# NVlabs/UnseenObjectClustering

Measured on AMD Instinct MI355X. Metric: frames/sec at 640x480 RGB-D, two-stage clustering, higher is better.
Workload: dtype f32; 1 GPU; configs[3] frames: full two-stage (crop-and-refine) segmentation of single 640x480 RGB-D frames; throughput schedule 3 streams x 4-frame launch sets (one frame at a time: `latency`); frame=640x480, seeds=100, iters=10, crop=224, total_frames=513, frames_per_gpu=513, collective=False, frames_in_flight_per_gpu=12, streams_per_gpu=3, frames_per_launch=4

## Files before the change

include/uoc_hip.h:

```cpp
#ifndef UOC_HIP_H
#define UOC_HIP_H

#include <stddef.h>
#include <stdint.h>

#ifdef __cplusplus
extern "C" {
#endif

#define UOC_OK 0
#define UOC_EINVAL (-22)
#define UOC_ENOMEM (-12)
#define UOC_EHIP (-5)
#define UOC_ENOENT (-2)
#define UOC_ETIMEDOUT (-110)

#define UOC_EMBED_DIM 64
#define UOC_MAX_SEEDS 128
#define UOC_METRIC_COSINE 0
#define UOC_METRIC_EUCLIDEAN 1

int uoc_version(void);
int uoc_is_dev_build(void);
unsigned long long uoc_config_fingerprint(void);
// ... 45 lines not shown
                     size_t ws_bytes, void *stream);
int uoc_ms_cluster_ex(const float *d_X, int batch, int n, int m, float kappa, int iters, float epsilon, int metric,
                      const int32_t *d_first_index, int32_t *d_labels, int32_t *d_indices, float *d_Z_out,
                      int32_t *d_seed_labels_out, void *d_ws, size_t ws_bytes, void *stream);
int uoc_ms_cluster_wide_ex(const float *d_X, int halves, int batch, int n, int m, float kappa, int iters, float epsilon,
                           int metric, const int32_t *d_first_index, int32_t *d_labels, int32_t *d_indices, float *d_Z_out,
                           int32_t *d_seed_labels_out, void *d_ws, size_t ws_bytes, void *stream);


typedef struct uoc_net uoc_net;

enum { UOC_NET_RGBD_ADD = 0, UOC_NET_COLOR = 1, UOC_NET_DEPTH = 2, UOC_NET_RGBD_EARLY = 3, UOC_NET_RGBD_CAT = 4 };

int uoc_net_create(uoc_net **out);
int uoc_net_create_mode(uoc_net **out, int mode);
int uoc_net_embed_dim(const uoc_net *net);
int uoc_net_destroy(uoc_net *net);
int uoc_net_load_param(uoc_net *net, const char *name, const float *host_data, size_t numel);
int uoc_net_finalize(uoc_net *net);
size_t uoc_net_workspace_bytes(const uoc_net *net, int B, int H, int W);
int uoc_net_set_split_precision(uoc_net *net, int on);
int uoc_net_forward(uoc_net *net, const float *d_rgb, const float *d_xyz, int B, int H, int W, float *d_embed,
                    void *d_ws, size_t ws_bytes, void *stream);

#define UOC_CONV_DIRECT 0
#define UOC_CONV_WINOGRAD4 4
#define UOC_CONV_WINOGRAD4_BF16X3 5
int uoc_conv2d_nhwc(const float *d_in, const float *d_w, const float *d_bias, const float *d_res, float *d_out,
                    int G, int B, int H, int W, int Cin, int Cout, int K, int stride, int dil, int pad, int relu,
                    void *stream);
int uoc_conv2d_nhwc_algo(const float *d_in, const float *d_w, const float *d_bias, const float *d_res, float *d_out,
                         int G, int B, int H, int W, int Cin, int Cout, int K, int stride, int dil, int pad, int relu,
                         int algo, void *stream);


typedef struct uoc_roi_table {
  int32_t K;
  int32_t label[128];
  int32_t box[128][4];
} uoc_roi_table;

size_t uoc_roi_workspace_bytes(void);

int uoc_prep_rgbd(const uint8_t *d_bgr, const uint16_t *d_depth_mm, int H, int W, float fx, float fy, float px,
                  float py, float mean_b, float mean_g, float mean_r, float *d_image, float *d_xyz, void *stream);

int uoc_filter_labels_depth(int32_t *d_labels, const float *d_z, long z_batch_stride, int B, int H, int W,
                            float threshold, void *d_ws, size_t ws_bytes, void *stream);

int uoc_roi_build(int32_t *d_labels, const float *d_z, int H, int W, float threshold, float pad_fraction,
                  uoc_roi_table *d_table, void *d_ws, size_t ws_bytes, void *stream);

int uoc_roi_crop(const float *d_rgb, const float *d_xyz, const int32_t *d_labels, int H, int W,
                 const uoc_roi_table *d_table, int K, int S, float *d_rgb_crops, float *d_xyz_crops,
                 float *d_mask_crops, void *stream);

int uoc_roi_match_stats(const int32_t *d_labels_crop, const float *d_mask_crops, const float *d_xyz_crops, int K,
                        int S, int32_t *d_keep, float *d_meanz, void *d_ws, size_t ws_bytes, void *stream);

int uoc_roi_paste(const int32_t *d_labels_crop, const uoc_roi_table *d_table, const int32_t *d_map,
                  const int32_t *d_order, int K, int S, int H, int W, int32_t *d_refined, void *stream);

int uoc_roi_match(const int32_t *d_labels_crop, const float *d_mask_crops, const float *d_xyz_crops,
                  const uoc_roi_table *d_table, int K, int S, int H, int W, int32_t *d_refined, int32_t *d_keep,
                  int32_t *d_plan, int32_t *d_status, void *d_ws, size_t ws_bytes, void *stream);

// ... 172 lines not shown
```

unseenobjectclustering_amd/_native.py:

```python
from __future__ import annotations

import ctypes
import os
from ctypes import c_char_p, c_float, c_int, c_int32, c_size_t, c_void_p, POINTER

from .build import LIB_PATH

_lib = None


class NativeError(RuntimeError):
    pass


def _declare(lib):
    P = c_void_p
    lib.uoc_version.restype = c_int
    lib.uoc_is_dev_build.argtypes = []
    lib.uoc_is_dev_build.restype = c_int
    lib.uoc_config_fingerprint.argtypes = []
    lib.uoc_config_fingerprint.restype = ctypes.c_ulonglong
    lib.uoc_shutdown.restype = c_int
    lib.uoc_reload_env.argtypes = []
    lib.uoc_reload_env.restype = c_int
# ... 13 lines not shown
    lib.uoc_ms_seed_components.argtypes = [P, c_int, c_int, c_float, P, P, P]
    lib.uoc_ms_assign.argtypes = [P, c_int, c_int, P, P, P, c_int, P, P, P, c_size_t, P]
    lib.uoc_ms_cluster.argtypes = [P, c_int, c_int, c_int, c_float, c_int, c_float, P, P, P, P, P, P, c_size_t, P]
    lib.uoc_ms_check.argtypes = [P]
    lib.uoc_ms_check.restype = c_int
    lib.uoc_ms_workspace_bytes_wide.restype = c_size_t
    lib.uoc_ms_workspace_bytes_wide.argtypes = [c_int, c_int, c_int, c_int]
    lib.uoc_ms_cluster_wide.argtypes = [P, c_int, c_int, c_int, c_int, c_float, c_int, c_float, P, P, P, P, P, P, c_size_t, P]
    lib.uoc_ms_cluster_wide.restype = c_int
    lib.uoc_ms_select_seeds_ex.argtypes = [P, c_int, c_int, c_int, c_int, P, P, P, c_int, P, c_size_t, P]
    lib.uoc_ms_hill_climb_ex.argtypes = [P, c_int, c_int, P, c_int, c_float, c_int, c_int, P, c_size_t, P]
    lib.uoc_ms_seed_components_ex.argtypes = [P, c_int, c_int, c_float, c_int, P, P, P]
    lib.uoc_ms_assign_ex.argtypes = [P, c_int, c_int, P, P, P, c_int, c_int, P, P, P, c_size_t, P]
    lib.uoc_ms_cluster_ex.argtypes = [P, c_int, c_int, c_int, c_float, c_int, c_float, c_int, P, P, P, P, P, P, c_size_t, P]
    lib.uoc_ms_cluster_wide_ex.argtypes = [P, c_int, c_int, c_int, c_int, c_float, c_int, c_float, c_int, P, P, P, P, P, P,
                                           c_size_t, P]
    for name in METRIC_SYMBOLS:
        getattr(lib, name).restype = c_int
    lib.uoc_net_embed_dim.argtypes = [P]
    lib.uoc_net_embed_dim.restype = c_int
    lib.uoc_net_create.argtypes = [POINTER(P)]
    lib.uoc_net_create_mode.argtypes = [POINTER(P), c_int]
    lib.uoc_net_destroy.argtypes = [P]
    lib.uoc_net_load_param.argtypes = [P, c_char_p, P, c_size_t]
    lib.uoc_net_finalize.argtypes = [P]
    lib.uoc_net_workspace_bytes.restype = c_size_t
    lib.uoc_net_workspace_bytes.argtypes = [P, c_int, c_int, c_int]
    lib.uoc_net_forward.argtypes = [P, P, P, c_int, c_int, c_int, P, P, c_size_t, P]
    lib.uoc_net_set_split_precision.argtypes = [P, c_int]
    lib.uoc_net_set_split_precision.restype = c_int
    lib.uoc_conv2d_nhwc.argtypes = [P, P, P, P, P] + [c_int] * 11 + [P]
    lib.uoc_conv2d_nhwc_algo.argtypes = [P, P, P, P, P] + [c_int] * 12 + [P]
    lib.uoc_conv2d_nhwc_algo.restype = c_int
    for name in ("uoc_net_create", "uoc_net_create_mode", "uoc_net_destroy", "uoc_net_load_param", "uoc_net_finalize", "uoc_net_forward",
                 "uoc_conv2d_nhwc"):
        getattr(lib, name).restype = c_int
    lib.uoc_eval_workspace_bytes.restype = c_size_t
    lib.uoc_eval_workspace_bytes.argtypes = [c_int, c_int]
    lib.uoc_eval_pair_stats.argtypes = [P, P, c_int, c_int, c_int, P, P, c_size_t, P]
    lib.uoc_eval_pair_stats.restype = c_int
    lib.uoc_roi_workspace_bytes.restype = c_size_t
    lib.uoc_roi_workspace_bytes.argtypes = []
    lib.uoc_prep_rgbd.argtypes = [P, P, c_int, c_int] + [c_float] * 7 + [P, P, P]
    lib.uoc_prep_rgbd.restype = c_int
    lib.uoc_filter_labels_depth.argtypes = [P, P, ctypes.c_long, c_int, c_int, c_int, c_float, P, c_size_t, P]
    lib.uoc_roi_build.argtypes = [P, P, c_int, c_int, c_float, c_float, P, P, c_size_t, P]
    lib.uoc_roi_crop.argtypes = [P, P, P, c_int, c_int, P, c_int, c_int, P, P, P, P]
    lib.uoc_roi_match_stats.argtypes = [P, P, P, c_int, c_int, P, P, P, c_size_t, P]
    lib.uoc_roi_paste.argtypes = [P, P, P, P, c_int, c_int, c_int, c_int, P, P]
    lib.uoc_labels_to_u8.argtypes = [P, ctypes.c_long, P, P, P]
    lib.uoc_roi_match.argtypes = [P, P, P, P, c_int, c_int, c_int, c_int, P, P, P, P, P, c_size_t, P]
    for name in ("uoc_filter_labels_depth", "uoc_roi_build", "uoc_roi_crop", "uoc_roi_match_stats", "uoc_roi_paste", "uoc_labels_to_u8", "uoc_roi_match"):
        getattr(lib, name).restype = c_int
    lib.uoc_objects_workspace_bytes.argtypes = [c_int, c_int, c_int]
    lib.uoc_objects_workspace_bytes.restype = c_size_t
    lib.uoc_objects.argtypes = [P, P, P, c_int, c_int, c_int, c_int, c_int, P, P, P, P, ctypes.c_long, P, P, c_size_t, P]
    lib.uoc_objects.restype = c_int
    lib.uoc_track_state_bytes.argtypes = [c_int, c_int, c_int]
    lib.uoc_track_state_bytes.restype = c_size_t
    lib.uoc_track_workspace_bytes.argtypes = [c_int]
    lib.uoc_track_workspace_bytes.restype = c_size_t
    lib.uoc_track_reset.argtypes = [P, c_int, c_int, c_int, c_int, P]
    lib.uoc_track_reset.restype = c_int
    lib.uoc_track_step.argtypes = [P, c_int, c_int, c_int, c_int, c_int, P, P, P, P, P, c_size_t, P]
    lib.uoc_track_step.restype = c_int
    lib.uoc_cc_workspace_bytes.argtypes = [c_int, c_int, c_int]
# ... 26 lines not shown
    lib.uoc_footprint.restype = c_int
    lib.uoc_lzf_decompress.argtypes = [P, c_size_t, P, c_size_t]
    lib.uoc_lzf_decompress.restype = ctypes.c_long
    lib.uoc_prof_enable.argtypes = [c_int]
    lib.uoc_prof_reset.argtypes = []
    lib.uoc_prof_report.argtypes = [ctypes.c_char_p, c_size_t]
    for name in ("uoc_prof_enable", "uoc_prof_reset", "uoc_prof_report"):
        getattr(lib, name).restype = c_int
    for name in ("uoc_ms_select_seeds", "uoc_ms_select_seeds_from", "uoc_ms_hill_climb", "uoc_ms_seed_components", "uoc_ms_assign",
                 "uoc_ms_cluster"):
        getattr(lib, name).restype = c_int


METRIC_COSINE = 0
METRIC_EUCLIDEAN = 1
METRICS = {"cosine": METRIC_COSINE, "euclidean": METRIC_EUCLIDEAN}
METRIC_SYMBOLS = ("uoc_ms_select_seeds_ex", "uoc_ms_hill_climb_ex", "uoc_ms_seed_components_ex", "uoc_ms_assign_ex",
                  "uoc_ms_cluster_ex", "uoc_ms_cluster_wide_ex")


def metric_code(metric) -> int:
    if metric not in METRICS:
        raise NotImplementedError(f"metric={metric!r}: only 'cosine' and 'euclidean' are implemented on gfx950")
    return METRICS[metric]


EXPORTED_SYMBOLS = (
    "uoc_version", "uoc_is_dev_build", "uoc_config_fingerprint", "uoc_shutdown", "uoc_last_error", "uoc_reload_env", "uoc_ms_set_persistent_fps", "uoc_ms_set_stream_ordering", "uoc_ms_fps_fallbacks", "uoc_ms_check", "uoc_ms_workspace_bytes", "uoc_ms_select_seeds", "uoc_ms_select_seeds_from", "uoc_ms_hill_climb",
    "uoc_ms_seed_components", "uoc_ms_assign", "uoc_ms_cluster", "uoc_ms_workspace_bytes_wide", "uoc_ms_cluster_wide",
) + METRIC_SYMBOLS + (
    "uoc_net_embed_dim",
    "uoc_net_create", "uoc_net_create_mode", "uoc_net_destroy", "uoc_net_load_param", "uoc_net_finalize", "uoc_net_workspace_bytes",
    "uoc_net_forward", "uoc_net_set_split_precision", "uoc_conv2d_nhwc", "uoc_conv2d_nhwc_algo",
    "uoc_roi_workspace_bytes", "uoc_prep_rgbd", "uoc_filter_labels_depth", "uoc_roi_build", "uoc_roi_crop", "uoc_roi_match_stats",
    "uoc_roi_paste", "uoc_roi_match", "uoc_labels_to_u8", "uoc_eval_workspace_bytes", "uoc_eval_pair_stats", "uoc_objects_workspace_bytes", "uoc_objects",
    "uoc_track_state_bytes", "uoc_track_workspace_bytes", "uoc_track_reset", "uoc_track_step",
    "uoc_cc_workspace_bytes", "uoc_cc_split", "uoc_plane_workspace_bytes", "uoc_support_plane",
    "uoc_relations_workspace_bytes", "uoc_relations", "uoc_placement_workspace_bytes", "uoc_placement",
    "uoc_grasp_workspace_bytes", "uoc_grasp", "uoc_elevation_workspace_bytes", "uoc_elevation",
    "uoc_footprint_workspace_bytes", "uoc_footprint", "uoc_lzf_decompress", "uoc_prof_enable", "uoc_prof_reset", "uoc_prof_report",
)


class RoiTable(ctypes.Structure):
    _fields_ = [("K", c_int32), ("label", c_int32 * 128), ("box", (c_int32 * 4) * 128)]


ROI_TABLE_BYTES = ctypes.sizeof(RoiTable)


class UocObject(ctypes.Structure):
    _fields_ = [("pixels", c_int32), ("count", c_int32), ("box", c_int32 * 4), ("centroid", c_float * 3), ("cov", c_float * 6),
                ("aabb_min", c_float * 3), ("aabb_max", c_float * 3), ("eig", c_float * 3), ("axes", c_float * 9),
                ("obb_center", c_float * 3), ("obb_half", c_float * 3), ("offset", c_int32), ("kept", c_int32)]


OBJECT_BYTES = ctypes.sizeof(UocObject)


class UocPlane(ctypes.Structure):
    _fields_ = [("found", c_int32), ("candidates", c_int32), ("inliers", c_int32), ("hyp", c_int32), ("normal", c_float * 3),
                ("d", c_float), ("centroid", c_float * 3), ("eig", c_float * 3), ("rms", c_float), ("u", c_float * 3),
                ("v", c_float * 3)]


class UocPlaneObject(ctypes.Structure):
# ... 32 lines not shown
FOOT_ROOMIEST, FOOT_NEAREST = 0, 1


class UocTrack(ctypes.Structure):
    _fields_ = [("uid", c_int32), ("age", c_int32), ("hits", c_int32), ("area", c_int32), ("born", c_int32)]


TRACK_FIELDS = tuple(name for name, _ in UocTrack._fields_)
TRACK_SLOTS = 128
TRACK_HEADER_WORDS = 1024
TRACK_META_WORD = 640
TRACK_CONT_WORDS = 128 * 128
CC_ALL, CC_LARGEST = 0, 1
CC_MODES = {"all": CC_ALL, "largest": CC_LARGEST}
CC_FIELDS = ("src", "area", "root", "siblings")
OBJECTS_MAX_ATTR = 8


def lib():
    global _lib
    if _lib is None:
        if not os.path.exists(LIB_PATH):
            raise NativeError(
                f"{LIB_PATH} not found: build it with `python -m unseenobjectclustering_amd.build` "
                "(or __graft_entry__.build()).  There is no CPU fallback.")
        import torch
        l = ctypes.CDLL(LIB_PATH)
        try:
            _declare(l)
        except AttributeError as e:
            raise NativeError(f"{LIB_PATH} lacks a symbol of include/uoc_hip.h ({e}): rebuild it with "
                              "`python -m unseenobjectclustering_amd.build`") from e
        _lib = l
        import atexit
        atexit.register(l.uoc_shutdown)
    return _lib


CONV_DIRECT, CONV_WINOGRAD4, CONV_WINOGRAD4_BF16X3 = 0, 4, 5


def config_fingerprint() -> int:
    return int(lib().uoc_config_fingerprint())


def check(rc: int, what: str):
    if rc != 0:
        msg = lib().uoc_last_error().decode("utf-8", "replace")
        raise NativeError(f"{what} failed (rc={rc}): {msg}")


def ptr(t):
    if t is None:
        return c_void_p(0)
    return c_void_p(t.data_ptr())


def stream_ptr(device=None):
    import torch
    return c_void_p(torch.cuda.current_stream(device).cuda_stream)


def stream_key(device):
    import torch
    return (device.type, device.index, int(torch.cuda.current_stream(device).cuda_stream))


_retired = []
GRAPHS_ALIVE = 0


def retire(t):
# ... 15 lines not shown
```

unseenobjectclustering_amd/csrc/conv.h:

```cpp
#pragma once
#include "common.h"

namespace uoc {

struct ConvParams {
  const float *in;
  const float *w;
  const float *bias;
  const float *res;
  float *out;
  int G, B, H, W, Cin, Ho, Wo, Cout;
  int KH, KW, stride, dil, pad, relu;
  int stem;
  int tune = 1;
  int prof_kc = -1;
  double prof_flops = 0.0;
  int prof_tag[4] = {0, 0, 0, 0};
};

int launch_conv(const ConvParams &p, hipStream_t st);


bool wino4_eligible(const ConvParams &p);
bool wino4_channels_ok(int Cin, int Cout);
size_t wino4_ws_floats(int G, int B, int H, int W, int d, int Cin, int Cout);
int launch_wino4_weights(const float *w, float *U, int G, int Cout, int Cin, hipStream_t st);
int launch_wino4_conv(const ConvParams &p, const float *U, float *ws, hipStream_t st, const unsigned short *U3 = nullptr);
int launch_wino4_split_weights(const float *U, unsigned short *U3, int G, int Cout, int Cin, hipStream_t st);
int launch_wino4_slice_split(const ConvParams &p0, int Bg, int b0, const unsigned short *U3, float *ws, hipStream_t st);
struct Wino4Geom;
int w4_stage_output(const ConvParams &p, const Wino4Geom &geo, const float *Mw, hipStream_t st);
long wino4_elem_blocks(long items);
int launch_nchw3_to_nhwc4(const float *in, float *out, int B, int H, int W, hipStream_t st);
int launch_maxpool3x3s2(const float *in, float *out, int n_img, int H, int W, int C, int Ho, int Wo, hipStream_t st);
int launch_head(const float *fa, const float *fb, float *embed, int B, int h, int w, int H, int W, int cat,
                hipStream_t st);

}
```

unseenobjectclustering_amd/csrc/net.hip:

```cpp
#include <map>
#include <mutex>
#include <string>
#include <vector>

#include "conv.h"

#include <stdlib.h>

namespace uoc {

struct ConvLayer {
  std::string conv, bn;
  int Cin, Cout, K, stride, dil, pad, relu;
  bool has_bn, has_bias, stem;
  float *d_w = nullptr, *d_b = nullptr;
  float *d_U4 = nullptr;
  unsigned short *d_U3 = nullptr;
  size_t w_per_group = 0;
};

struct Block {
  int conv1, conv2, down;
};

// ... 308 lines not shown
  UOC_REQUIRE(B >= 1 && H >= 8 && W >= 8, "bad input shape B=%d H=%d W=%d", B, H, W);
  const int G = n->G;
  const NetWs w = carve_net(d_ws, n->mode, n->wino_f, B, H, W);
  UOC_REQUIRE(d_ws && ws_bytes >= w.total && ((uintptr_t)d_ws & 255) == 0, "workspace too small or misaligned (%zu < %zu)",
              ws_bytes, w.total);
  hipStream_t st = (hipStream_t)stream;
  const Dims d = dims(H, W);

  const ConvLayer &stem = n->layers[n->stem];
  const size_t in_stride = (size_t)B * H * W * 4;
  if (n->mode == UOC_NET_RGBD_EARLY) {
    if (int rc = launch_nchw3_to_nhwc4(d_rgb, w.in4, B, H, W, st)) return rc;
    if (int rc = launch_nchw3_to_nhwc4(d_xyz, w.in4 + in_stride, B, H, W, st)) return rc;
    ConvLayer part = stem;
    part.d_w = stem.d_w + stem.w_per_group;
    part.d_b = stem.d_b + (size_t)G * stem.Cout;
    part.relu = 0;
    if (int rc = run_conv(1, part, w.in4 + in_stride, nullptr, w.stem_part, B, H, W, d.H1, d.W1, st)) return rc;
    if (int rc = run_conv(1, stem, w.in4, w.stem_part, w.stem, B, H, W, d.H1, d.W1, st)) return rc;
  } else {
    const float *first = n->mode == UOC_NET_DEPTH ? d_xyz : d_rgb;
    if (int rc = launch_nchw3_to_nhwc4(first, w.in4, B, H, W, st)) return rc;
    if (G == 2)
      if (int rc = launch_nchw3_to_nhwc4(d_xyz, w.in4 + in_stride, B, H, W, st)) return rc;
    if (int rc = run_conv(G, stem, w.in4, nullptr, w.stem, B, H, W, d.H1, d.W1, st)) return rc;
  }
  if (int rc = launch_maxpool3x3s2(w.stem, w.buf[0], G * B, d.H1, d.W1, 64, d.H2, d.W2, st)) return rc;

  int cur = 0, h = d.H2, wd = d.W2;
  for (const Block &b : n->blocks) {
    const ConvLayer &c1 = n->layers[b.conv1], &c2 = n->layers[b.conv2];
    const int ho = (h - 1) / c1.stride + 1, wo = (wd - 1) / c1.stride + 1;
    float *x = w.buf[cur], *tmp = w.buf[(cur + 1) & 3], *sc = w.buf[(cur + 2) & 3], *y = w.buf[(cur + 3) & 3];
    if (int rc = run_conv(G, c1, x, nullptr, tmp, B, h, wd, ho, wo, st, w.wino, n->split)) return rc;
    const float *res = x;
    if (b.down >= 0) {
      if (int rc = run_conv(G, n->layers[b.down], x, nullptr, sc, B, h, wd, ho, wo, st)) return rc;
      res = sc;
    }
    if (int rc = run_conv(G, c2, tmp, res, y, B, ho, wo, ho, wo, st, w.wino, n->split)) return rc;
    cur = (cur + 3) & 3;
    h = ho;
    wd = wo;
  }
  if (int rc = run_conv(G, n->layers[n->fc], w.buf[cur], nullptr, w.fc, B, h, wd, h, wd, st)) return rc;
  return launch_head(w.fc, G == 2 ? w.fc + (size_t)B * h * wd * 64 : nullptr, d_embed, B, h, wd, H, W,
                     n->mode == UOC_NET_RGBD_CAT, st);
}

int uoc_conv2d_nhwc_algo(const float *d_in, const float *d_w, const float *d_bias, const float *d_res, float *d_out, int G,
                         int B, int H, int W, int Cin, int Cout, int K, int stride, int dil, int pad, int relu, int algo,
                         void *stream) {
  UOC_REQUIRE(K == 1 || K == 3, "K=%d (only 1 or 3)", K);
  UOC_REQUIRE(d_res == nullptr || d_res != d_out, "conv2d: the residual must not alias the output");
  ConvParams p;
  p.tune = 0;
  p.in = d_in;
  p.w = d_w;
  p.bias = d_bias;
  p.res = d_res;
  p.out = d_out;
  p.G = G;
  p.B = B;
  p.H = H;
  p.W = W;
  p.Cin = Cin;
// ... 12 lines not shown
  std::lock_guard<std::mutex> lock(mu);
  if (algo == UOC_CONV_WINOGRAD4 || algo == UOC_CONV_WINOGRAD4_BF16X3) {
    UOC_REQUIRE(wino4_eligible(p), "conv2d: shape not eligible for Winograd F(4x4,3x3)");
    static float *U4 = nullptr, *ws4 = nullptr;
    static unsigned short *U3 = nullptr;
    static size_t ucap4 = 0, wcap4 = 0, ucap3 = 0;
    const size_t un = (size_t)G * 36 * Cout * Cin, wn = wino4_ws_floats(G, B, H, W, dil, Cin, Cout);
    if (un > ucap4) {
      if (U4) (void)hipFree(U4);
      UOC_HIP_CHECK(hipMalloc(&U4, un * sizeof(float)));
      ucap4 = un;
    }
    if (wn > wcap4) {
      if (ws4) (void)hipFree(ws4);
      UOC_HIP_CHECK(hipMalloc(&ws4, wn * sizeof(float)));
      wcap4 = wn;
    }
    if (int rc = launch_wino4_weights(d_w, U4, G, Cout, Cin, st)) return rc;
    if (algo == UOC_CONV_WINOGRAD4_BF16X3) {
      if (3 * un > ucap3) {
        if (U3) (void)hipFree(U3);
        UOC_HIP_CHECK(hipMalloc(&U3, 3 * un * sizeof(unsigned short)));
        ucap3 = 3 * un;
      }
      if (int rc = launch_wino4_split_weights(U4, U3, G, Cout, Cin, st)) return rc;
      return launch_wino4_conv(p, U4, ws4, st, U3);
    }
    return launch_wino4_conv(p, U4, ws4, st);
  }
  set_error("conv2d: unknown algorithm %d", algo);
  return UOC_EINVAL;
}

int uoc_conv2d_nhwc(const float *d_in, const float *d_w, const float *d_bias, const float *d_res, float *d_out, int G,
                    int B, int H, int W, int Cin, int Cout, int K, int stride, int dil, int pad, int relu,
                    void *stream) {
  return uoc_conv2d_nhwc_algo(d_in, d_w, d_bias, d_res, d_out, G, B, H, W, Cin, Cout, K, stride, dil, pad, relu,
                              UOC_CONV_DIRECT, stream);
}

}
```

unseenobjectclustering_amd/csrc/prof.h:

```cpp
#pragma once
#include <hip/hip_runtime.h>

namespace uoc {

enum KernelClass {
  KC_CONV_160x128 = 0,
  KC_CONV_80x128,
  KC_CONV_160x64,
  KC_CONV_80x64,
  KC_CONV_STEM,
  KC_GLDS_160x128,
  KC_GLDS_80x128,
  KC_GLDS_160x64,
  KC_GLDS_80x64,
  KC_WINO_INPUT,
  KC_WINO_GEMM,
  KC_NET_MISC,
  KC_HEAD,
  KC_FPS_STEP,
  KC_HC_ITER,
  KC_HC_FINALIZE,
  KC_SEED_CC,
  KC_ASSIGN,
  KC_RELABEL,
  KC_ROI,
  KC_WINO4_INPUT,
  KC_WINO4_GEMM,
  KC_WINO4_OUTPUT,
  KC_PLANE_CAND,
  KC_PLANE_HYP,
  KC_PLANE_SCORE,
  KC_PLANE_REFINE,
  KC_PLANE_OBJECTS,
  KC_REL_PAIRS,
  KC_REL_DERIVE,
  KC_PLACE_RASTER,
  KC_PLACE_TRANSFORM,
  KC_GRASP_MOMENTS,
  KC_GRASP_CANDIDATES,
  KC_ELEV_RASTER,
  KC_ELEV_TRANSFORM,
  KC_FOOT_TABLES,
  KC_FOOT_FIT,
  KC_COUNT
};

struct ProfTag {
  int v[4] = {0, 0, 0, 0};
};

extern bool g_prof_enabled;
void prof_begin(int kc, hipStream_t st, double flops, double bytes, const ProfTag &tag);
void prof_end(hipStream_t st);

struct ProfScope {
  hipStream_t st;
  bool on;
  ProfScope(int kc, hipStream_t s, double flops, double bytes, const ProfTag &tag = ProfTag()) : st(s), on(g_prof_enabled) {
    if (on) prof_begin(kc, s, flops, bytes, tag);
  }
  ~ProfScope() {
    if (on) prof_end(st);
  }
};

}
```

unseenobjectclustering_amd/csrc/prof.hip:

```cpp
#include "prof.h"

#include <stdio.h>
#include <string.h>

#include <vector>

#include "common.h"

namespace uoc {

bool g_prof_enabled = false;

static const char *kNames[KC_COUNT] = {
    "conv_mfma_160x128", "conv_mfma_80x128", "conv_mfma_160x64", "conv_mfma_80x64", "conv_stem",
    "conv_glds_160x128", "conv_glds_80x128", "conv_glds_160x64", "conv_glds_80x64",
    "wino_input",        "wino_gemm",
    "net_misc",          "head",             "fps_step",         "hc_iter",         "hc_finalize",
    "seed_cc",           "assign",           "relabel",          "roi",
    "wino4_input",       "wino4_gemm",       "wino4_output",
    "plane_candidates",  "plane_hypotheses", "plane_score",      "plane_refine",    "plane_objects",
    "relations_pairs",   "relations_derive",
    "placement_raster",  "placement_transform",
    "grasp_moments",     "grasp_candidates",
    "elevation_raster",  "elevation_transform",
    "footprint_tables",  "footprint_fit"};

struct Rec {
  int kc;
  hipEvent_t a, b;
  double flops, bytes;
  ProfTag tag;
};
static std::vector<Rec> g_recs;
static std::vector<hipEvent_t> g_pool;

static hipEvent_t get_event() {
  if (!g_pool.empty()) {
    hipEvent_t e = g_pool.back();
    g_pool.pop_back();
    return e;
  }
  hipEvent_t e;
  (void)hipEventCreate(&e);
  return e;
}

void prof_begin(int kc, hipStream_t st, double flops, double bytes, const ProfTag &tag) {
  Rec r;
  r.kc = kc;
  r.a = get_event();
  r.b = get_event();
  r.flops = flops;
  r.bytes = bytes;
  r.tag = tag;
  (void)hipEventRecord(r.a, st);
  g_recs.push_back(r);
}

// ... 83 lines not shown
```

unseenobjectclustering_amd/csrc/wino4.hip:

```cpp
#include "conv.h"
#include "dma.h"
#include "prof.h"
#include "wino4_math.h"

#include <stdlib.h>

namespace uoc {

constexpr int W4BK = 32;
#ifndef W4_OUT_MIN_BLOCKS
#define W4_OUT_MIN_BLOCKS 2
#endif

__global__ __launch_bounds__(256) void wino4_weight_kernel(const float *__restrict__ w, float *__restrict__ U, int G,
                                                           int Cout, int Cin) {
  const long total = (long)G * Cout * Cin;
  for (long i = (long)blockIdx.x * blockDim.x + threadIdx.x; i < total; i += (long)gridDim.x * blockDim.x) {
    const int ci = (int)(i % Cin);
    const int co = (int)((i / Cin) % Cout);
    const int g = (int)(i / ((long)Cin * Cout));
    wino4_weight_body(w, U, G, Cout, Cin, g, co, ci);
  }
}

template <int VEC>
__global__ __launch_bounds__(256) void wino4_input_kernel(const float *__restrict__ in, float *__restrict__ V,
                                                          Wino4Geom geo, int G, int C) {
  const int CV = C / VEC;
  const long total = (long)G * geo.NT * CV;
#ifndef W4_IN_XCD
#define W4_IN_XCD 1
#endif
  const long vblock = W4_IN_XCD ? (long)(blockIdx.x & 7) * (gridDim.x >> 3) + (blockIdx.x >> 3) : (long)blockIdx.x;
  for (long idx = vblock * blockDim.x + threadIdx.x; idx < total; idx += (long)gridDim.x * blockDim.x) {
    const int cv = (int)(idx % CV);
    const int tau = (int)((idx / CV) % geo.NT);
    const int g = (int)(idx / ((long)CV * geo.NT));
    wino4_input_body<VEC>(in, V, geo, C, g, tau, cv);
  }
}

template <int VEC>
__global__ __launch_bounds__(256, W4_OUT_MIN_BLOCKS) void wino4_output_kernel(const float *__restrict__ M, const float *__restrict__ bias,
                                                           const float *__restrict__ res, float *__restrict__ out,
                                                           Wino4Geom geo, int G, int Cout, int relu) {
  const int CV = Cout / VEC;
  const long total = (long)G * geo.NT * CV;
  for (long idx = (long)blockIdx.x * blockDim.x + threadIdx.x; idx < total; idx += (long)gridDim.x * blockDim.x) {
    const int cv = (int)(idx % CV);
    const int tau = (int)((idx / CV) % geo.NT);
    const int g = (int)(idx / ((long)CV * geo.NT));
    wino4_output_body<VEC>(M, bias, res, out, geo, Cout, relu, g, tau, cv);
  }
}



__device__ __forceinline__ f32x4 w4mfma(float a, float b, f32x4 c) {
  return __builtin_amdgcn_mfma_f32_16x16x4f32(a, b, c, 0, 0, 0);
}

#ifndef UOC_W4_ABLATE
#define UOC_W4_ABLATE 0
#endif
#define W4_BARRIER() do { if (UOC_W4_ABLATE != 1) __builtin_amdgcn_s_barrier(); } while (0)
template <int N>
__device__ __forceinline__ void w4_wait_vmcnt() {
  if (UOC_W4_ABLATE != 2) wait_vmcnt<N>();
}

template <int BM, int BN, bool PAIR, int NW>
__global__ __launch_bounds__(NW * 64) void wino4_gemm_kernel(const float *__restrict__ V, const float *__restrict__ U,
                                                             float *__restrict__ Mo, int NT, int Cin, int Cout, int planes,
                                                             int mtiles, int nt_shift) {
  static_assert(NW == 8 || NW == 4, "waves per block");
  constexpr int WAVES_N = NW / 2;
  constexpr int WM = BM / 2, WN = BN / WAVES_N;
  constexpr int TM = WM / 16, TN = WN / 16;
  constexpr int R = BM + BN;
  constexpr int RPP = NW * 8;
  constexpr int NPA = (BM + RPP - 1) / RPP, NPW = (BN + RPP - 1) / RPP, NPASS = NPA + NPW;
  constexpr int STAGE = R * W4BK;
  static_assert(WM % 16 == 0 && WN % 16 == 0 && R % 8 == 0 && NPASS <= 12, "tile shape");

  extern __shared__ __attribute__((aligned(16))) float smem[];

// ... 311 lines not shown
bool wino4_channels_ok(int Cin, int Cout) {
  const int n64 = Cout / 64;
  return Cin % W4BK == 0 && Cout % 64 == 0 && n64 > 0 && (n64 & (n64 - 1)) == 0;
}

bool wino4_eligible(const ConvParams &p) {
  return !p.stem && p.KH == 3 && p.KW == 3 && p.stride == 1 && p.pad == p.dil && wino4_channels_ok(p.Cin, p.Cout) &&
         p.Ho == p.H && p.Wo == p.W;
}

size_t wino4_ws_floats(int G, int B, int H, int W, int d, int Cin, int Cout) {
  const Wino4Geom geo = make_geom4(B, H, W, d);
  return (size_t)G * 36 * geo.NT * 5 / 2 * (size_t)(Cin > Cout ? Cin : Cout) + 64;
}

int launch_wino4_weights(const float *w, float *U, int G, int Cout, int Cin, hipStream_t st) {
  const long total = (long)G * Cout * Cin;
  long blocks = (total + 255) / 256;
  if (blocks > 4096) blocks = 4096;
  hipLaunchKernelGGL(wino4_weight_kernel, dim3((unsigned)blocks), dim3(256), 0, st, w, U, G, Cout, Cin);
  UOC_LAUNCH_CHECK();
  return UOC_OK;
}

long wino4_elem_blocks(long items) {
  long blocks = (items + 255) / 256;
  const long cap = 16384;
  blocks = blocks < cap ? blocks : cap;
  return (blocks + 7) / 8 * 8;
}

static int launch_wino4_slice(const ConvParams &p0, int Bg, int b0, const float *U, float *ws, hipStream_t st);

int launch_wino4_conv(const ConvParams &p, const float *U, float *ws, hipStream_t st, const unsigned short *U3) {
  UOC_REQUIRE(wino4_eligible(p), "winograd F(4x4): layer not eligible");
  UOC_REQUIRE(U && ws && p.in && p.out, "winograd F(4x4): null tensor/weight/workspace pointer");
  const int planes = 36 * p.G;
  UOC_REQUIRE((size_t)planes * p.Cout * p.Cin * 4 < (1ull << 32), "winograd F(4x4): weight planes exceed 4 GB");
  const size_t per_image = (size_t)planes * make_geom4(1, p.H, p.W, p.dil).NT * (p.Cin > p.Cout ? p.Cin : p.Cout) * (U3 ? 6 : 4);
  UOC_REQUIRE(per_image < (1ull << 32), "winograd F(4x4): one image's frequency planes exceed 4 GB");
  static EnvInt limit_mb("UOC_SPLIT_MAX_MB", 0);
  const size_t limit = limit_mb.get() > 0 && ((size_t)limit_mb.get() << 20) > per_image ? (size_t)limit_mb.get() << 20 : (1ull << 32) - 1;
  const int bmax = (int)(limit / per_image);
  if (p.B > bmax) {
    for (int b0 = 0; b0 < p.B; b0 += bmax) {
      ConvParams q = p;
      q.B = p.B - b0 < bmax ? p.B - b0 : bmax;
      if (int rc = U3 ? launch_wino4_slice_split(q, p.B, b0, U3, ws, st) : launch_wino4_slice(q, p.B, b0, U, ws, st)) return rc;
    }
    return UOC_OK;
  }
  return U3 ? launch_wino4_slice_split(p, p.B, 0, U3, ws, st) : launch_wino4_slice(p, p.B, 0, U, ws, st);
}

static int w4_vec() { return 4; }

static int w4_stage_input(const ConvParams &p, const Wino4Geom &geo, float *V, hipStream_t st) {
  const double Mpix = (double)p.B * p.H * p.W;
  const ProfTag tag = {{geo.NT, p.Cin, p.Cout, p.dil}};
  const int vec = w4_vec();
  ProfScope prof(KC_WINO4_INPUT, st, 0.0, 4.0 * p.G * (Mpix * p.Cin + 36.0 * geo.NT * p.Cin), tag);
  const long blocks = wino4_elem_blocks((long)p.G * geo.NT * (p.Cin / vec));
    hipLaunchKernelGGL(wino4_input_kernel<4>, dim3((unsigned)blocks), dim3(256), 0, st, p.in, V, geo, p.G, p.Cin);
  UOC_LAUNCH_CHECK();
  return UOC_OK;
}

static int w4_stage_gemm(const ConvParams &p, const Wino4Geom &geo, const float *U, float *V, float *Mw, hipStream_t st) {
  const int planes = 36 * p.G;
  const double Mpix = (double)p.B * p.H * p.W;
  const ProfTag tag = {{geo.NT, p.Cin, p.Cout, p.dil}};
  const double gflops = 2.0 * Mpix * p.Cout * p.Cin * 9.0 * p.G;
  const double gbytes = 4.0 * planes * ((double)geo.NT * p.Cin + (double)p.Cout * p.Cin + (double)geo.NT * p.Cout);
  ProfScope prof(KC_WINO4_GEMM, st, gflops, gbytes, tag);
  return launch_wino4_gemm(V, U, Mw, geo.NT, p.Cin, p.Cout, planes, st);
}

int w4_stage_output(const ConvParams &p, const Wino4Geom &geo, const float *Mw, hipStream_t st) {
  const double Mpix = (double)p.B * p.H * p.W;
  const ProfTag tag = {{geo.NT, p.Cin, p.Cout, p.dil}};
  const int vec = w4_vec();
  ProfScope prof(KC_WINO4_OUTPUT, st, 0.0, 4.0 * p.G * (36.0 * geo.NT * p.Cout + Mpix * p.Cout * (p.res ? 2 : 1)), tag);
  const long blocks = wino4_elem_blocks((long)p.G * geo.NT * (p.Cout / vec));
    hipLaunchKernelGGL(wino4_output_kernel<4>, dim3((unsigned)blocks), dim3(256), 0, st, Mw, p.bias, p.res, p.out, geo, p.G, p.Cout, p.relu);
  UOC_LAUNCH_CHECK();
  return UOC_OK;
}

static int launch_wino4_slice(const ConvParams &p0, int Bg, int b0, const float *U, float *ws, hipStream_t st) {
  ConvParams p = p0;
  const size_t img_in = (size_t)p.H * p.W * p.Cin, img_out = (size_t)p.H * p.W * p.Cout;
  p.in += (size_t)b0 * img_in;
  p.out += (size_t)b0 * img_out;
  if (p.res) p.res += (size_t)b0 * img_out;
  Wino4Geom geo = make_geom4(p.B, p.H, p.W, p.dil);
  geo.Bg = Bg;
  float *V = ws, *Mw = ws + (size_t)36 * p.G * geo.NT * p.Cin;
  if (int rc = w4_stage_input(p, geo, V, st)) return rc;
  if (int rc = w4_stage_gemm(p, geo, U, V, Mw, st)) return rc;
  return w4_stage_output(p, geo, Mw, st);
}

}
```

unseenobjectclustering_amd/csrc/wino4_math.h:

```cpp
#pragma once
#include <hip/hip_runtime.h>

namespace uoc {

struct Wino4Geom {
  int B, H, W, d, TH, TW, NT;
  int Bg;
};

__host__ __device__ inline Wino4Geom make_geom4(int B, int H, int W, int d) {
  Wino4Geom g;
  g.B = B;
  g.H = H;
  g.W = W;
  g.d = d;
  g.TH = ((H + d - 1) / d + 3) / 4;
  g.TW = ((W + d - 1) / d + 3) / 4;
  g.NT = B * d * d * g.TH * g.TW;
  g.Bg = B;
  return g;
}

__host__ __device__ inline void wino4_decode(int tau, const Wino4Geom &g, int &b, int &oy, int &ox) {
  const int tx = tau % g.TW;
// ... 211 lines not shown
      T col[6], o[4];
#pragma unroll
      for (int i = 0; i < 6; ++i) col[i] = m[6 * i + j];
      wino4_at(col, o);
#pragma unroll
      for (int a = 0; a < 4; ++a) s[a][j] = o[a];
    }
    if (W4_OUT_RES_MODE == 2) { W4_LOAD_RES() }
#pragma unroll
    for (int a = 0; a < 4; ++a) wino4_at(s[a], yv[a]);
  }
#undef W4_LOAD_RES
  T bv;
  if (bias)
    bv = *reinterpret_cast<const T *>(bias + (size_t)g * Cout + VEC * cv);
  else
    w4_zero(bv);
#pragma unroll
  for (int a = 0; a < 4; ++a) {
    const int y = oy + a * geo.d;
    if (y >= geo.H) continue;
#pragma unroll
    for (int e = 0; e < 4; ++e) {
      const int x = ox + e * geo.d;
      if (x >= geo.W) continue;
      T v = w4_add(yv[a][e], bv);
      if (res) v = w4_add(v, W4_OUT_RES_MODE == 0 ? *reinterpret_cast<const T *>(res + o0 + a * oy_step + e * ox_step) : rv[a][e]);
      if (relu) v = w4_relu(v);
      *reinterpret_cast<T *>(out + o0 + a * oy_step + e * ox_step) = v;
    }
  }
}

}
```

Baseline: 175.4 frames/s.

## Fuse Winograd output and next-layer input transforms for residual block conv pairs

Adds a fused mid-stage kernel that takes the first conv's Winograd output tiles, applies bias, residual and ReLU, keeps the spatial result in LDS, and emits the second conv's Winograd input tiles directly. This skips writing and re-reading the intermediate activation in global memory and removes one launch per residual block. An auto heuristic enables it only for small grids where the elementwise kernels underfill the CUs, and only when the spatial plane fits in 64KB of LDS. The risks are lower parallelism, since each block covers a whole image slice, and heavy register use from the 36-element tiles.

```diff
diff --git a/include/uoc_hip.h b/include/uoc_hip.h
--- a/include/uoc_hip.h
+++ b/include/uoc_hip.h
@@ -101,6 +101,11 @@
 int uoc_conv2d_nhwc_algo(const float *d_in, const float *d_w, const float *d_bias, const float *d_res, float *d_out,
                          int G, int B, int H, int W, int Cin, int Cout, int K, int stride, int dil, int pad, int relu,
                          int algo, void *stream);
+int uoc_wino4_set_fuse(int mode);
+int uoc_wino4_fused_launches(void);
+int uoc_conv2d_pair_nhwc(const float *d_in, const float *d_w1, const float *d_b1, const float *d_res1, int relu1,
+                         const float *d_w2, const float *d_b2, const float *d_res2, int relu2, float *d_mid, float *d_out,
+                         int G, int B, int H, int W, int C0, int C1, int C2, int dil, int keep_mid, void *stream);
 
 
 typedef struct uoc_roi_table {
diff --git a/unseenobjectclustering_amd/_native.py b/unseenobjectclustering_amd/_native.py
--- a/unseenobjectclustering_amd/_native.py
+++ b/unseenobjectclustering_amd/_native.py
@@ -69,6 +69,12 @@
     lib.uoc_conv2d_nhwc.argtypes = [P, P, P, P, P] + [c_int] * 11 + [P]
     lib.uoc_conv2d_nhwc_algo.argtypes = [P, P, P, P, P] + [c_int] * 12 + [P]
     lib.uoc_conv2d_nhwc_algo.restype = c_int
+    lib.uoc_wino4_set_fuse.argtypes = [c_int]
+    lib.uoc_wino4_set_fuse.restype = c_int
+    lib.uoc_wino4_fused_launches.argtypes = []
+    lib.uoc_wino4_fused_launches.restype = c_int
+    lib.uoc_conv2d_pair_nhwc.argtypes = [P, P, P, P, c_int, P, P, P, c_int, P, P] + [c_int] * 9 + [P]
+    lib.uoc_conv2d_pair_nhwc.restype = c_int
     for name in ("uoc_net_create", "uoc_net_create_mode", "uoc_net_destroy", "uoc_net_load_param", "uoc_net_finalize", "uoc_net_forward",
                  "uoc_conv2d_nhwc"):
         getattr(lib, name).restype = c_int
@@ -161,6 +167,7 @@
     "uoc_net_embed_dim",
     "uoc_net_create", "uoc_net_create_mode", "uoc_net_destroy", "uoc_net_load_param", "uoc_net_finalize", "uoc_net_workspace_bytes",
     "uoc_net_forward", "uoc_net_set_split_precision", "uoc_conv2d_nhwc", "uoc_conv2d_nhwc_algo",
+    "uoc_wino4_set_fuse", "uoc_wino4_fused_launches", "uoc_conv2d_pair_nhwc",
     "uoc_roi_workspace_bytes", "uoc_prep_rgbd", "uoc_filter_labels_depth", "uoc_roi_build", "uoc_roi_crop", "uoc_roi_match_stats",
     "uoc_roi_paste", "uoc_roi_match", "uoc_labels_to_u8", "uoc_eval_workspace_bytes", "uoc_eval_pair_stats", "uoc_objects_workspace_bytes", "uoc_objects",
     "uoc_track_state_bytes", "uoc_track_workspace_bytes", "uoc_track_reset", "uoc_track_step",
@@ -259,12 +266,21 @@
             raise NativeError(f"{LIB_PATH} lacks a symbol of include/uoc_hip.h ({e}): rebuild it with "
                               "`python -m unseenobjectclustering_amd.build`") from e
         _lib = l
+        set_wino4_fuse(os.environ.get("UOC_WINO4_FUSE", "auto"))
         import atexit
         atexit.register(l.uoc_shutdown)
     return _lib
 
 
 CONV_DIRECT, CONV_WINOGRAD4, CONV_WINOGRAD4_BF16X3 = 0, 4, 5
+WINO4_FUSE_MODES = {"auto": -1, "": -1, "0": 0, "1": 1}
+
+
+def set_wino4_fuse(mode):
+    key = str(mode).strip().lower()
+    if key not in WINO4_FUSE_MODES:
+        raise ValueError(f"UOC_WINO4_FUSE={mode!r}: expected auto, 0 or 1")
+    check(lib().uoc_wino4_set_fuse(WINO4_FUSE_MODES[key]), "uoc_wino4_set_fuse")
 
 
 def config_fingerprint() -> int:
diff --git a/unseenobjectclustering_amd/csrc/conv.h b/unseenobjectclustering_amd/csrc/conv.h
--- a/unseenobjectclustering_amd/csrc/conv.h
+++ b/unseenobjectclustering_amd/csrc/conv.h
@@ -26,6 +26,11 @@
 size_t wino4_ws_floats(int G, int B, int H, int W, int d, int Cin, int Cout);
 int launch_wino4_weights(const float *w, float *U, int G, int Cout, int Cin, hipStream_t st);
 int launch_wino4_conv(const ConvParams &p, const float *U, float *ws, hipStream_t st, const unsigned short *U3 = nullptr);
+int wino4_pair_slice(const ConvParams &p1, const ConvParams &p2);
+int launch_wino4_pair(const ConvParams &p1, const ConvParams &p2, const float *U1, const float *U2, float *ws, bool keep_mid,
+                      hipStream_t st);
+int wino4_set_fuse_mode(int mode);
+int wino4_fused_launches();
 int launch_wino4_split_weights(const float *U, unsigned short *U3, int G, int Cout, int Cin, hipStream_t st);
 int launch_wino4_slice_split(const ConvParams &p0, int Bg, int b0, const unsigned short *U3, float *ws, hipStream_t st);
 struct Wino4Geom;
diff --git a/unseenobjectclustering_amd/csrc/net.hip b/unseenobjectclustering_amd/csrc/net.hip
--- a/unseenobjectclustering_amd/csrc/net.hip
+++ b/unseenobjectclustering_amd/csrc/net.hip
@@ -364,6 +364,19 @@
     const ConvLayer &c1 = n->layers[b.conv1], &c2 = n->layers[b.conv2];
     const int ho = (h - 1) / c1.stride + 1, wo = (wd - 1) / c1.stride + 1;
     float *x = w.buf[cur], *tmp = w.buf[(cur + 1) & 3], *sc = w.buf[(cur + 2) & 3], *y = w.buf[(cur + 3) & 3];
+    if (c1.d_U4 && c2.d_U4 && w.wino && !n->split) {
+      const ConvParams p1 = conv_params(G, c1, x, nullptr, tmp, B, h, wd, ho, wo);
+      const ConvParams p2 = conv_params(G, c2, tmp, b.down >= 0 ? sc : x, y, B, ho, wo, ho, wo);
+      if (wino4_pair_slice(p1, p2) > 0) {
+        if (b.down >= 0)
+          if (int rc = run_conv(G, n->layers[b.down], x, nullptr, sc, B, h, wd, ho, wo, st)) return rc;
+        if (int rc = launch_wino4_pair(p1, p2, c1.d_U4, c2.d_U4, w.wino, false, st)) return rc;
+        cur = (cur + 3) & 3;
+        h = ho;
+        wd = wo;
+        continue;
+      }
+    }
     if (int rc = run_conv(G, c1, x, nullptr, tmp, B, h, wd, ho, wo, st, w.wino, n->split)) return rc;
     const float *res = x;
     if (b.down >= 0) {
@@ -442,6 +455,48 @@
   return UOC_EINVAL;
 }
 
+int uoc_wino4_set_fuse(int mode) { return wino4_set_fuse_mode(mode); }
+int uoc_wino4_fused_launches(void) { return wino4_fused_launches(); }
+
+int uoc_conv2d_pair_nhwc(const float *d_in, const float *d_w1, const float *d_b1, const float *d_res1, int relu1, const float *d_w2,
+                         const float *d_b2, const float *d_res2, int relu2, float *d_mid, float *d_out, int G, int B, int H, int W,
+                         int C0, int C1, int C2, int dil, int keep_mid, void *stream) {
+  UOC_REQUIRE(d_in && d_w1 && d_w2 && d_mid && d_out, "conv2d_pair: null tensor pointer");
+  UOC_REQUIRE(G >= 1 && B >= 1 && H >= 1 && W >= 1 && dil >= 1, "conv2d_pair: bad shape G=%d B=%d H=%d W=%d dil=%d", G, B, H, W, dil);
+  UOC_REQUIRE(d_mid != d_out && d_res1 != d_mid && d_res2 != d_out, "conv2d_pair: aliased tensors");
+  ConvParams p1;
+  p1.tune = 0;
+  p1.in = d_in, p1.w = d_w1, p1.bias = d_b1, p1.res = d_res1, p1.out = d_mid;
+  p1.G = G, p1.B = B, p1.H = p1.Ho = H, p1.W = p1.Wo = W, p1.Cin = C0, p1.Cout = C1;
+  p1.KH = p1.KW = 3, p1.stride = 1, p1.dil = p1.pad = dil, p1.relu = relu1, p1.stem = 0;
+  ConvParams p2 = p1;
+  p2.in = d_mid, p2.w = d_w2, p2.bias = d_b2, p2.res = d_res2, p2.out = d_out;
+  p2.Cin = C1, p2.Cout = C2, p2.relu = relu2;
+  UOC_REQUIRE(wino4_eligible(p1) && wino4_eligible(p2), "conv2d_pair: shape not eligible for Winograd F(4x4,3x3)");
+  hipStream_t st = (hipStream_t)stream;
+  static std::mutex mu;
+  std::lock_guard<std::mutex> lock(mu);
+  static float *U = nullptr, *ws = nullptr;
+  static size_t ucap = 0, wcap = 0;
+  const size_t u1 = (size_t)G * 36 * C1 * C0, u2 = (size_t)G * 36 * C2 * C1;
+  const size_t wa = wino4_ws_floats(G, B, H, W, dil, C0, C1), wb = wino4_ws_floats(G, B, H, W, dil, C1, C2), wn = wa > wb ? wa : wb;
+  if (u1 + u2 > ucap) {
+    if (U) (void)hipFree(U);
+    ucap = 0;
+    UOC_HIP_CHECK(hipMalloc(&U, (u1 + u2) * sizeof(float)));
+    ucap = u1 + u2;
+  }
+  if (wn > wcap) {
+    if (ws) (void)hipFree(ws);
+    wcap = 0;
+    UOC_HIP_CHECK(hipMalloc(&ws, wn * sizeof(float)));
+    wcap = wn;
+  }
+  if (int rc = launch_wino4_weights(d_w1, U, G, C1, C0, st)) return rc;
+  if (int rc = launch_wino4_weights(d_w2, U + u1, G, C2, C1, st)) return rc;
+  return launch_wino4_pair(p1, p2, U, U + u1, ws, keep_mid != 0, st);
+}
+
 int uoc_conv2d_nhwc(const float *d_in, const float *d_w, const float *d_bias, const float *d_res, float *d_out, int G,
                     int B, int H, int W, int Cin, int Cout, int K, int stride, int dil, int pad, int relu,
                     void *stream) {
diff --git a/unseenobjectclustering_amd/csrc/prof.h b/unseenobjectclustering_amd/csrc/prof.h
--- a/unseenobjectclustering_amd/csrc/prof.h
+++ b/unseenobjectclustering_amd/csrc/prof.h
@@ -42,6 +42,7 @@
   KC_ELEV_TRANSFORM,
   KC_FOOT_TABLES,
   KC_FOOT_FIT,
+  KC_WINO4_MID,
   KC_COUNT
 };
 
diff --git a/unseenobjectclustering_amd/csrc/prof.hip b/unseenobjectclustering_amd/csrc/prof.hip
--- a/unseenobjectclustering_amd/csrc/prof.hip
+++ b/unseenobjectclustering_amd/csrc/prof.hip
@@ -23,7 +23,7 @@
     "placement_raster",  "placement_transform",
     "grasp_moments",     "grasp_candidates",
     "elevation_raster",  "elevation_transform",
-    "footprint_tables",  "footprint_fit"};
+    "footprint_tables",  "footprint_fit",    "wino4_mid"};
 
 struct Rec {
   int kc;
diff --git a/unseenobjectclustering_amd/csrc/wino4.hip b/unseenobjectclustering_amd/csrc/wino4.hip
--- a/unseenobjectclustering_amd/csrc/wino4.hip
+++ b/unseenobjectclustering_amd/csrc/wino4.hip
@@ -52,6 +52,25 @@
     const int g = (int)(idx / ((long)CV * geo.NT));
     wino4_output_body<VEC>(M, bias, res, out, geo, Cout, relu, g, tau, cv);
   }
+}
+
+constexpr int W4_MID_VEC = 2;
+constexpr int W4_MID_MAX_THREADS = 512;
+__global__ __launch_bounds__(W4_MID_MAX_THREADS) void wino4_mid_kernel(const float *__restrict__ M, const float *__restrict__ bias,
+                                                                       const float *__restrict__ res, float *__restrict__ yout,
+                                                                       float *__restrict__ V, Wino4Geom geo, int C, int relu, int CS) {
+  typedef W4Vec<W4_MID_VEC>::type T;
+  extern __shared__ __attribute__((aligned(16))) float w4_mid_lds[];
+  T *ysm = reinterpret_cast<T *>(w4_mid_lds);
+  const Wino4Unit u = wino4_unit((int)blockIdx.x, geo, C, CS);
+  const int Q = CS / W4_MID_VEC;
+  const int items = geo.TH * geo.TW * Q, cells = (4 * geo.TH + 2) * (4 * geo.TW + 2) * Q;
+  const int tid = threadIdx.x, nthr = blockDim.x;
+  for (int i = tid; i < cells; i += nthr) w4_zero(ysm[i]);
+  __syncthreads();
+  for (int it = tid; it < items; it += nthr) wino4_mid_output_item<W4_MID_VEC>(M, bias, res, yout, ysm, geo, C, relu, u, it / Q, it % Q);
+  __syncthreads();
+  for (int it = tid; it < items; it += nthr) wino4_mid_input_item<W4_MID_VEC>(ysm, V, geo, C, u, it / Q, it % Q);
 }
 
 
@@ -429,16 +448,22 @@
 
 static int launch_wino4_slice(const ConvParams &p0, int Bg, int b0, const float *U, float *ws, hipStream_t st);
 
+static int w4_batch_limit(const ConvParams &p, bool split) {
+  const size_t per_image = (size_t)36 * p.G * make_geom4(1, p.H, p.W, p.dil).NT * (p.Cin > p.Cout ? p.Cin : p.Cout) * (split ? 6 : 4);
+  if (per_image >= (1ull << 32)) return 0;
+  static EnvInt limit_mb("UOC_SPLIT_MAX_MB", 0);
+  const size_t limit = limit_mb.get() > 0 && ((size_t)limit_mb.get() << 20) > per_image ? (size_t)limit_mb.get() << 20 : (1ull << 32) - 1;
+  return (int)(limit / per_image);
+}
+
+
 int launch_wino4_conv(const ConvParams &p, const float *U, float *ws, hipStream_t st, const unsigned short *U3) {
   UOC_REQUIRE(wino4_eligible(p), "winograd F(4x4): layer not eligible");
   UOC_REQUIRE(U && ws && p.in && p.out, "winograd F(4x4): null tensor/weight/workspace pointer");
   const int planes = 36 * p.G;
   UOC_REQUIRE((size_t)planes * p.Cout * p.Cin * 4 < (1ull << 32), "winograd F(4x4): weight planes exceed 4 GB");
-  const size_t per_image = (size_t)planes * make_geom4(1, p.H, p.W, p.dil).NT * (p.Cin > p.Cout ? p.Cin : p.Cout) * (U3 ? 6 : 4);
-  UOC_REQUIRE(per_image < (1ull << 32), "winograd F(4x4): one image's frequency planes exceed 4 GB");
-  static EnvInt limit_mb("UOC_SPLIT_MAX_MB", 0);
-  const size_t limit = limit_mb.get() > 0 && ((size_t)limit_mb.get() << 20) > per_image ? (size_t)limit_mb.get() << 20 : (1ull << 32) - 1;
-  const int bmax = (int)(limit / per_image);
+  const int bmax = w4_batch_limit(p, U3 != nullptr);
+  UOC_REQUIRE(bmax > 0, "winograd F(4x4): one image's frequency planes exceed 4 GB");
   if (p.B > bmax) {
     for (int b0 = 0; b0 < p.B; b0 += bmax) {
       ConvParams q = p;
@@ -482,6 +507,80 @@
     hipLaunchKernelGGL(wino4_output_kernel<4>, dim3((unsigned)blocks), dim3(256), 0, st, Mw, p.bias, p.res, p.out, geo, p.G, p.Cout, p.relu);
   UOC_LAUNCH_CHECK();
   return UOC_OK;
+}
+
+constexpr int kW4FuseMinCs = 32;
+constexpr int kW4FuseMaxLds = 64 * 1024;
+constexpr int kW4ElemBlocksPerCu = 2;
+static std::atomic<int> g_w4_fuse_mode{-1};
+static std::atomic<int> g_w4_fused_launches{0};
+
+int wino4_set_fuse_mode(int mode) {
+  UOC_REQUIRE(mode >= -1 && mode <= 1, "winograd F(4x4): fuse mode %d (-1 auto, 0 off, 1 on)", mode);
+  g_w4_fuse_mode.store(mode);
+  return UOC_OK;
+}
+int wino4_fused_launches() { return g_w4_fused_launches.load(); }
+
+static int pick_wino4_fuse(const Wino4Geom &geo, int G, int C) {
+  const int mode = g_w4_fuse_mode.load();
+  if (mode == 0) return 0;
+  if (mode < 0) {
+    const int ncu = device_num_cu() > 0 ? device_num_cu() : 256;
+    if ((long)G * geo.NT * (C / 4) > (long)ncu * kW4ElemBlocksPerCu * 256) return 0;
+  }
+  const long cells = (long)(4 * geo.TH + 2) * (4 * geo.TW + 2), tiles = (long)geo.TH * geo.TW;
+  int best = 0;
+  for (int cs = kW4FuseMinCs; cs <= 128; cs <<= 1) {
+    if (C % cs || cells * cs * 4 > kW4FuseMaxLds) break;
+    if (best == 0 || tiles * (cs / W4_MID_VEC) <= 256) best = cs;
+  }
+  return best;
+}
+
+int wino4_pair_slice(const ConvParams &p1, const ConvParams &p2) {
+  if (!wino4_eligible(p1) || !wino4_eligible(p2)) return 0;
+  if (p1.G != p2.G || p1.B != p2.B || p1.H != p2.H || p1.W != p2.W || p1.dil != p2.dil || p1.Cout != p2.Cin || p1.out != p2.in) return 0;
+  if ((size_t)36 * p1.G * p1.Cout * p1.Cin * 4 >= (1ull << 32) || (size_t)36 * p2.G * p2.Cout * p2.Cin * 4 >= (1ull << 32)) return 0;
+  if (p1.B > w4_batch_limit(p1, false) || p2.B > w4_batch_limit(p2, false)) return 0;
+  return pick_wino4_fuse(make_geom4(p1.B, p1.H, p1.W, p1.dil), p1.G, p1.Cout);
+}
+
+static int w4_stage_mid(const ConvParams &p1, const Wino4Geom &geo, int cs, bool keep_mid, const float *Mw, float *V, hipStream_t st) {
+  const int C = p1.Cout;
+  const int units = p1.G * p1.B * p1.dil * p1.dil * (C / cs);
+  const int items = geo.TH * geo.TW * (cs / W4_MID_VEC);
+  int threads = (items + 63) / 64 * 64;
+  if (threads > W4_MID_MAX_THREADS) threads = W4_MID_MAX_THREADS;
+  const size_t lds = (size_t)(4 * geo.TH + 2) * (4 * geo.TW + 2) * cs * sizeof(float);
+  UOC_REQUIRE(cs >= W4_MID_VEC && C % cs == 0 && lds <= (size_t)kW4FuseMaxLds, "winograd F(4x4): fused transform with %d channels per block", cs);
+  const double Mpix = (double)p1.B * p1.H * p1.W;
+  const ProfTag tag = {{geo.NT, C, C, p1.dil}};
+  ProfScope prof(KC_WINO4_MID, st, 0.0, 4.0 * p1.G * (72.0 * geo.NT * C + Mpix * C * ((p1.res ? 1 : 0) + (keep_mid ? 1 : 0))), tag);
+  hipLaunchKernelGGL(wino4_mid_kernel, dim3((unsigned)units), dim3(threads), lds, st, Mw, p1.bias, p1.res, keep_mid ? p1.out : nullptr, V,
+                     geo, C, p1.relu, cs);
+  UOC_LAUNCH_CHECK();
+  g_w4_fused_launches.fetch_add(1);
+  return UOC_OK;
+}
+
+int launch_wino4_pair(const ConvParams &p1, const ConvParams &p2, const float *U1, const float *U2, float *ws, bool keep_mid,
+                      hipStream_t st) {
+  const int cs = wino4_pair_slice(p1, p2);
+  if (cs == 0) {
+    if (int rc = launch_wino4_conv(p1, U1, ws, st)) return rc;
+    return launch_wino4_conv(p2, U2, ws, st);
+  }
+  UOC_REQUIRE(U1 && U2 && ws && p1.in && p1.out && p2.out, "winograd F(4x4): null tensor/weight/workspace pointer");
+  const Wino4Geom geo = make_geom4(p1.B, p1.H, p1.W, p1.dil);
+  int cmax = p1.Cin > p1.Cout ? p1.Cin : p1.Cout;
+  if (p2.Cout > cmax) cmax = p2.Cout;
+  float *V = ws, *Mw = ws + (size_t)36 * p1.G * geo.NT * cmax;
+  if (int rc = w4_stage_input(p1, geo, V, st)) return rc;
+  if (int rc = w4_stage_gemm(p1, geo, U1, V, Mw, st)) return rc;
+  if (int rc = w4_stage_mid(p1, geo, cs, keep_mid, Mw, V, st)) return rc;
+  if (int rc = w4_stage_gemm(p2, geo, U2, V, Mw, st)) return rc;
+  return w4_stage_output(p2, geo, Mw, st);
 }
 
 static int launch_wino4_slice(const ConvParams &p0, int Bg, int b0, const float *U, float *ws, hipStream_t st) {
diff --git a/unseenobjectclustering_amd/csrc/wino4_math.h b/unseenobjectclustering_amd/csrc/wino4_math.h
--- a/unseenobjectclustering_amd/csrc/wino4_math.h
+++ b/unseenobjectclustering_amd/csrc/wino4_math.h
@@ -267,4 +267,85 @@
   }
 }
 
-}
+struct Wino4Unit {
+  int g, b, py, px, ch0, CS;
+};
+
+__host__ __device__ inline Wino4Unit wino4_unit(int unit, const Wino4Geom &geo, int C, int CS) {
+  Wino4Unit u;
+  const int slices = C / CS;
+  u.CS = CS;
+  u.ch0 = (unit % slices) * CS;
+  unit /= slices;
+  u.px = unit % geo.d;
+  unit /= geo.d;
+  u.py = unit % geo.d;
+  unit /= geo.d;
+  u.b = unit % geo.B;
+  u.g = unit / geo.B;
+  return u;
+}
+
+__host__ __device__ inline int wino4_unit_tile0(const Wino4Unit &u, const Wino4Geom &geo) {
+  return ((u.b * geo.d + u.py) * geo.d + u.px) * geo.TH * geo.TW;
+}
+
+template <int VEC>
+__host__ __device__ inline void wino4_mid_output_item(const float *M, const float *bias, const float *res, float *yout,
+                                                      typename W4Vec<VEC>::type *ysm, const Wino4Geom &geo, int C, int relu,
+                                                      const Wino4Unit &u, int t, int cq) {
+  typedef typename W4Vec<VEC>::type T;
+  const int Q = u.CS / VEC, Wl = 4 * geo.TW + 2;
+  const int ty = t / geo.TW, tx = t - ty * geo.TW;
+  const int ch = u.ch0 + VEC * cq;
+  const size_t plane = (size_t)geo.NT * C;
+  const float *src = M + (size_t)u.g * 36 * plane + (size_t)(wino4_unit_tile0(u, geo) + t) * C + ch;
+  T m[36];
+#pragma unroll
+  for (int k = 0; k < 36; ++k) m[k] = W4_STREAM_LOAD(T, src + (size_t)k * plane);
+  T yv[4][4];
+  wino4_output_tile(m, yv);
+  T bv;
+  if (bias)
+    bv = *reinterpret_cast<const T *>(bias + (size_t)u.g * C + ch);
+  else
+    w4_zero(bv);
+  const size_t gsz = (size_t)geo.Bg * geo.H * geo.W * C;
+#pragma unroll
+  for (int a = 0; a < 4; ++a) {
+    const int y = u.py + (4 * ty + a) * geo.d;
+    if (y >= geo.H) continue;
+#pragma unroll
+    for (int e = 0; e < 4; ++e) {
+      const int x = u.px + (4 * tx + e) * geo.d;
+      if (x >= geo.W) continue;
+      const size_t o = (size_t)u.g * gsz + (((size_t)u.b * geo.H + y) * geo.W + x) * C + ch;
+      T v = w4_add(yv[a][e], bv);
+      if (res) v = w4_add(v, *reinterpret_cast<const T *>(res + o));
+      if (relu) v = w4_relu(v);
+      ysm[((4 * ty + a + 1) * Wl + 4 * tx + e + 1) * Q + cq] = v;
+      if (yout) *reinterpret_cast<T *>(yout + o) = v;
+    }
+  }
+}
+
+template <int VEC>
+__host__ __device__ inline void wino4_mid_input_item(const typename W4Vec<VEC>::type *ysm, float *V, const Wino4Geom &geo, int C,
+                                                     const Wino4Unit &u, int t, int cq) {
+  typedef typename W4Vec<VEC>::type T;
+  const int Q = u.CS / VEC, Wl = 4 * geo.TW + 2;
+  const int ty = t / geo.TW, tx = t - ty * geo.TW;
+  T d[6][6];
+#pragma unroll
+  for (int i = 0; i < 6; ++i)
+#pragma unroll
+    for (int j = 0; j < 6; ++j) d[i][j] = ysm[((4 * ty + i) * Wl + 4 * tx + j) * Q + cq];
+  T v[36];
+  wino4_input_tile(d, v);
+  const size_t plane = (size_t)geo.NT * C;
+  float *dst = V + (size_t)u.g * 36 * plane + (size_t)(wino4_unit_tile0(u, geo) + t) * C + u.ch0 + VEC * cq;
+#pragma unroll
+  for (int k = 0; k < 36; ++k) W4_STREAM_STORE(T, dst + (size_t)k * plane, v[k]);
+}
+
+}
```

After: 175.9 frames/s, median of 3. About the same (+0.3%).
